# SoraKurihara/FFM

Measured on AMD Instinct MI355X. Metric: agent-steps/sec (whole node), 12×12 grid × 64k envs, 1/2/4/8 GPU, higher is better.
Workload: dtype f32; 1 GPU; ffm_core step, 12x12 room, 32 agents/env, 65536 envs/GPU, neumann, Philox seed 42, on-device auto-reset, steady state (envs desynchronised by a 1000-step untimed burn-in after reset); burn_in_steps=1000, map=12x12, agents_per_env=32, envs_per_gpu=65536, global_envs=65536, parallelism=env-sharded x1

## Files before the change

### ffm_amd/csrc/core_multi.hip

```cpp
#include <hip/hip_runtime.h>
#include <stdint.h>

#include "core_common.h"
#include "kernels.h"
#include "lane_common.h"
#include "episode_log.h"
#include "wave_reset.h"

namespace ffm {

namespace {

struct MultiCarve {
    size_t grid, tile, words, keys, posb, per_wave;
};

__host__ __device__ inline MultiCarve multi_carve(int PHW, int TS, int F) {
    MultiCarve c;
    size_t o = 0;
    c.grid = o;  o += a16((size_t)(2 * PHW) * 2);
    c.tile = o;  o += a16((size_t)(2 * TS) * 4);
    c.words = o; o += 64 * 8;
    c.keys = o;  o += a16((size_t)(F > 0 ? F : 1) * 8);
    c.posb = o;  o += 64 * 2;
// ... 115 lines not shown
                                   ((slot <= (uint32_t)NB ? slot : DirCodes::kNoDir) << 8));
            wave_sync();

            const int r = (int)slot_cell<NB>(slot, pp, PW);
            const bool req = slot <= (uint32_t)NB;
            const bool moving = req && r != pp;
            bool granted = req && !moving;
            {
                const int rt = moving ? r : pp;
                int m = 0, kr = 0, o = 0x7F;
#pragma unroll
                for (int s = 0; s < NB; s++) {
                    const uint32_t c = gk[rt - nb_dx<NB>(s) * PW - nb_dy<NB>(s)];
                    const bool is = (c & DirCodes::kAgent) != 0u && ((c >> 8) & 0xFu) == (uint32_t)s;
                    const int who = (int)(c & DirCodes::kIdx);
                    m += is ? 1 : 0;
                    kr += (is && who < al) ? 1 : 0;
                    o = (is && who < o) ? who : o;
                }
                if (moving) {
                    if (m == 1) {
                        granted = true;
                    } else {
                        const uint2 f = words[sub * 32 + o];
                        const int kk = philox_friction(f.x, f.y, (uint32_t)m, a.key0, a.key1, t, genv, (uint32_t)o);
                        granted = kk == kr;
                    }
                }
            }
            if (granted) __hip_atomic_fetch_add(dk + pp + dd0, 1.0f, __ATOMIC_RELAXED, __HIP_MEMORY_SCOPE_WAVEFRONT);
            const int np = granted ? r : pp;

            const bool keep = live && !(granted && to_exit);
            const unsigned long long km = __ballot(keep);
            const unsigned long long segm = sub ? 0xFFFFFFFF00000000ull : 0x00000000FFFFFFFFull;
            const int newidx = lanes_below(km & segm);
            const int newcnt = __popcll(km & segm);
            {
                const int n0 = __popcll(km & 0xFFFFFFFFull), n1 = __popcll(km >> 32);
                const int c0 = __builtin_amdgcn_readlane(cnt, 0), c1 = __builtin_amdgcn_readlane(cnt, 32);
                c_exits += (unsigned)((c0 - n0) + (nenv > 1 ? c1 - n1 : 0));
            }
            if (live) *mine = 0;
            if (keep) posb[sub * 32 + newidx] = (uint16_t)unpad(np, PW);
            const bool rs = a.auto_reset && env_ok && newcnt == 0;
            const unsigned long long rsm = __ballot(rs);
            if (rsm) {
                c_resets += (unsigned)(((rsm & 1ull) ? 1 : 0) + ((rsm >> 32) & 1ull ? 1 : 0));
                if (a.episodes && al == 0 && rs) a.episodes[e0 + sub] += 1;
                CoreStepArgs ak = a;
                ak.t = t;
                wave_sync();
                for (int s = 0; s < 2; s++)
                    if ((rsm >> (32 * s)) & 1ull) wave_reset_env(ak, ebase + (uint32_t)(e0 + s), keys, pfree, posb + s * 32, lane);
            }
            if (EPL && (rsm || !a.auto_reset))
                eplog_end_wave(a, env_ok && al == 0 && newcnt == 0 && cnt > 0, rs && al == 0, e0 + sub, t, lane);
            cnt = rs ? a.N : newcnt;
            wave_sync();
            cpos = posb[lane];

            auto stencil = [&](int tb, bool yl, bool yr, float4& out) {
                const float* p = tile + tb;
                float b[3][6];
#pragma unroll
                for (int dx = -1; dx <= 1; dx++) {
                    const float4 u = *reinterpret_cast<const float4*>(p + dx * W);
                    b[dx + 1][1] = a.c0 * u.x; b[dx + 1][2] = a.c0 * u.y;
                    b[dx + 1][3] = a.c0 * u.z; b[dx + 1][4] = a.c0 * u.w;
                    if (NB == 4 && dx != 0) continue;
                    b[dx + 1][0] = a.c0 * tile[yl ? 0 : tb + dx * W - 1];
                    b[dx + 1][5] = a.c0 * tile[yr ? 0 : tb + dx * W + 4];
                }
                float ov[4];
#pragma unroll
                for (int j = 0; j < 4; j++) {
                    float acc = b[1][j + 1];
#pragma unroll
                    for (int s = 0; s < NB; s++) {
                        const float tt = a.c1 * b[1 + nb_dx<NB>(s)][j + 1 + nb_dy<NB>(s)];
                        acc = acc + tt;
                    }
                    ov[j] = acc < 1e-4f ? 0.0f : acc;
                }
                out = make_float4(ov[0], ov[1], ov[2], ov[3]);
            };
            o0 = make_float4(0.f, 0.f, 0.f, 0.f);
            o1 = o0;
            if (tb0 >= 0) stencil(tb0, yl0, yr0, o0);
            if (tb1 >= 0) stencil(tb1, yl1, yr1, o1);
            {
                const bool r0 = (rsm & 1ull) != 0, r1 = (rsm >> 32) != 0;
                const bool z0 = zs0 == 0 ? r0 : (zs0 == 1 && r1), z1 = zs1 == 0 ? r0 : (zs1 == 1 && r1);
                if (z0) o0 = make_float4(0.f, 0.f, 0.f, 0.f);
                if (z1) o1 = make_float4(0.f, 0.f, 0.f, 0.f);
            }
            wave_sync();
            if (tb0 >= 0) *reinterpret_cast<float4*>(tile + tb0) = o0;
            if (tb1 >= 0) *reinterpret_cast<float4*>(tile + tb1) = o1;
            wave_sync();
        }

        __builtin_amdgcn_raw_buffer_store_b16((uint16_t)cpos, rp, (env_ok && al < cnt) ? (sub * A + al) * 2 : kOOB, 0, 0);
        __builtin_amdgcn_raw_buffer_store_b32((unsigned)cnt, rc, al == 0 ? sub * 4 : kOOB, 0, 0);
        buf_st4(rd, 16 * lane, o0);
        buf_st4(rd, 16 * lane + 1024, o1);
    }
// ... 50 lines not shown
```

### ffm_amd/csrc/engine.cpp

```cpp
#include "../../include/ffm_amd.h"

#include <hip/hip_runtime.h>

#include <algorithm>
#include <cmath>
#include <cstdio>
#include <cstdlib>
#include <cstring>
#include <string>
#include <vector>

#include "kernels.h"

namespace {
thread_local std::string g_err;
}

namespace ffm {
int set_error(int code, const std::string& msg) {
    g_err = msg;
    return code;
}
}

namespace {

int fail(int code, const std::string& msg) { return ffm::set_error(code, msg); }

#define HIP_TRY(expr)                                                                           \
    do {                                                                                        \
        hipError_t e_ = (expr);                                                                 \
        if (e_ != hipSuccess)                                                                   \
            return fail(FFM_E_HIP, std::string(#expr) + ": " + hipGetErrorString(e_));          \
    } while (0)

}

struct ffm_engine {
    ffm_engine_desc d{};
    int HW = 0, F = 0, K = 1, block = 256;
    bool f64 = false, mt = false;
    bool lane = false;
    bool wave = false;
    int wave_blocks = 0;
    int lane_blocks = 0;
    bool group = false;
    int group_blocks = 0;
    int group_g = 4;
    bool multi = false;
    int multi_blocks = 0;
    int fused = 1;
    float kS32 = 0, kD32 = 0, c0 = 0, c1 = 0;
    double kS64 = 0;
    uint32_t t = 0;
    uint8_t* d_map = nullptr;
    void* d_sff = nullptr;
    uint16_t* d_free = nullptr;
    uint16_t* d_free_padded = nullptr;
    unsigned char* d_stage = nullptr;
    size_t stage_bytes = 0;
    int stage_q4 = 0;
    uint16_t* d_pos = nullptr;
    int32_t* d_cnt = nullptr;
    float* d_dff = nullptr;
    float* d_tmp = nullptr;
    int32_t* d_eps = nullptr;
    unsigned long long* d_ctr = nullptr;
    size_t ctr_slots = 1;
    uint32_t* d_mt_np = nullptr;
    uint32_t* d_mt_py = nullptr;
    unsigned long long* d_dbg = nullptr;
    bool big = false;
    bool block_reset = false;
    unsigned char* d_scratch = nullptr;
    size_t scratch_stride = 0;
    ffm::CoreCapture cap{};
    uint32_t* d_ep_start = nullptr;
    int32_t* d_eplog = nullptr;
    unsigned long long* d_eplog_n = nullptr;
    long long eplog_cap = 0;
    unsigned long long* d_ephist = nullptr;
    int ephist_bins = 0;
    struct Shard {
        long long e0 = 0, n = 0;
        int blocks = 0, g = 4;
        size_t ctr0 = 0;
    };
    std::vector<Shard> shards;
    hipStream_t sh_stream[3] = {nullptr, nullptr, nullptr};
    hipEvent_t sh_fork = nullptr;
    hipEvent_t sh_end[3] = {nullptr, nullptr, nullptr};
};

static constexpr int kMaxStepShards = 4;
static constexpr int kDefaultStepShards = 2;

static size_t ep_sum_offset(int bins) { return ((size_t)bins + 15) & ~(size_t)15; }
static size_t ep_stats_words(int bins) { return ep_sum_offset(bins) + (size_t)ffm::kEpSumSlots * ffm::kEpSumStride; }

static void free_episode_log(ffm_engine* e, bool ep_start_too) {
    (void)hipFree(e->d_eplog);
    (void)hipFree(e->d_eplog_n);
    (void)hipFree(e->d_ephist);
    e->d_eplog = nullptr;
    e->d_eplog_n = nullptr;
    e->d_ephist = nullptr;
    e->eplog_cap = 0;
    e->ephist_bins = 0;
    if (ep_start_too) {
        (void)hipFree(e->d_ep_start);
        e->d_ep_start = nullptr;
    }
}

// ... 24 lines not shown
    (void)hipFree(e->d_free_padded);
    (void)hipFree(e->d_stage);
    (void)hipFree(e->d_pos);
    (void)hipFree(e->d_cnt);
    (void)hipFree(e->d_dff);
    (void)hipFree(e->d_tmp);
    (void)hipFree(e->d_eps);
    (void)hipFree(e->d_ctr);
    (void)hipFree(e->d_mt_np);
    (void)hipFree(e->d_mt_py);
    (void)hipFree(e->d_dbg);
    (void)hipFree(e->d_scratch);
    free_capture(e);
    free_episode_log(e, true);
    delete e;
}

int ffm_engine_create(const ffm_engine_desc* desc, ffm_engine** out) {
    if (!desc || !out) return fail(FFM_E_INVALID, "null argument");
    *out = nullptr;
    const ffm_engine_desc& d = *desc;
    if (d.abi_version != FFM_ABI_VERSION) return fail(FFM_E_INVALID, "abi_version mismatch");
    if (d.variant != FFM_VARIANT_CORE) return fail(FFM_E_UNSUPPORTED, "only FFM_VARIANT_CORE is built");
    if (d.H < 3 || d.W < 3 || (long long)d.H * d.W > 65536)
        return fail(FFM_E_INVALID, "map must be at least 3x3 and at most 65536 cells");
    if (!ffm::magic_div_ok((uint64_t)(d.H + 2) * (d.W + 2), (uint32_t)d.W + 2u))
        return fail(FFM_E_INVALID, "map too large for the kernels' magic divisors");
    if (!d.map || !d.sff) return fail(FFM_E_INVALID, "map and sff are required");
    if (d.neighborhood != 4 && d.neighborhood != 8) return fail(FFM_E_INVALID, "neighborhood must be 4 or 8");
    if (d.sff_dtype != FFM_SFF_F32 && d.sff_dtype != FFM_SFF_F64) return fail(FFM_E_INVALID, "sff_dtype");
    if (d.n_envs < 1) return fail(FFM_E_INVALID, "n_envs must be >= 1");
    if (d.agent_capacity < 1 || d.agent_capacity > 32767) return fail(FFM_E_INVALID, "agent_capacity");
    if (d.n_agents < 0 || d.n_agents > d.agent_capacity) return fail(FFM_E_INVALID, "n_agents > agent_capacity");
    if (d.rng_mode != FFM_RNG_PHILOX && d.rng_mode != FFM_RNG_MT) return fail(FFM_E_INVALID, "rng_mode");
    const int H = d.H, W = d.W, HW = H * W;
    std::vector<uint16_t> fl;
    for (int i = 0; i < HW; i++) {
        const int x = i / W, y = i % W;
        const bool border = x == 0 || y == 0 || x == H - 1 || y == W - 1;
        if (d.map[i] == 0) {
            if (border) return fail(FFM_E_INVALID, "free cell on the map border (walls must enclose the room)");
            fl.push_back((uint16_t)i);
        }
    }
    if (d.n_agents > (int)fl.size())
        return fail(FFM_E_INVALID, "Cannot take a larger sample than population when 'replace=False'");

    ffm_engine* e = new ffm_engine();
    e->d = d;
    e->d.map = nullptr;
    e->d.sff = nullptr;
    e->HW = HW;
    e->F = (int)fl.size();
    e->f64 = d.sff_dtype == FFM_SFF_F64;
    e->mt = d.rng_mode == FFM_RNG_MT;
    e->kS32 = (float)(-d.k_S);
    e->kD32 = (float)d.k_D;
    e->kS64 = -d.k_S;
    e->c0 = (float)((1.0 - d.decay) * (1.0 - d.diffuse));
    e->c1 = (float)(d.decay * (1.0 - d.diffuse) / (double)d.neighborhood);

    auto cleanup = [&](int rc) {
        release(e);
        return rc;
    };
    hipError_t he = hipSetDevice(d.device);
    if (he != hipSuccess) return cleanup(fail(FFM_E_HIP, std::string("hipSetDevice: ") + hipGetErrorString(he)));

    const int A = d.agent_capacity;
    const bool reset_lds = !e->mt && d.auto_reset;
    const int EW = A <= 32 ? 2 : 1;
    const bool lane_ok = !e->mt && !e->f64 && A <= 32 && W % 4 == 0 && HW <= 256 &&
                         ((long long)d.n_envs + 7) * HW * 4 < (1ll << 31);
    e->group = (d.envs_per_block == 0 || d.envs_per_block == -3) && lane_ok && ffm::core_group_supported(H, W) &&
               ffm::core_group_smem_bytes(H, W, e->F, 4) <= 64 * 1024;
    e->multi = lane_ok && ffm::core_multi_smem_bytes(H, W, e->F, 4) <= 64 * 1024;
    e->lane = !e->group && (d.envs_per_block == 0 || d.envs_per_block == -2) && lane_ok &&
              ffm::core_lane_smem_bytes(H, W, e->F, 4) <= 64 * 1024;
    e->wave = !e->lane && !e->group && (d.envs_per_block == 0 || d.envs_per_block == -1) && A <= 64 && !e->f64 && W % 4 == 0 && EW * HW <= 512 &&
              ffm::core_wave_smem_bytes(H, W, A, e->F, e->mt, reset_lds, 4) <= 64 * 1024;
    e->block = A > 256 ? 512 : 256;
    if (const char* bs = getenv("FFM_BLOCK_BS"))
        if (atoi(bs) == 256 || atoi(bs) == 512) e->block = atoi(bs);
    int K = d.envs_per_block > 0 ? d.envs_per_block : std::max(1, 256 / A);
    if (e->mt) K = 1;
    while (K > 1 && ffm::core_block_smem_bytes(H, W, A, K, e->F, e->f64, e->mt, reset_lds) > 64 * 1024) K--;
    e->K = K;
    e->big = !e->wave && !e->lane && !e->group &&
             ((size_t)(H + 2) * (W + 2) > 65535 ||
              ffm::core_block_smem_bytes(H, W, A, K, e->F, e->f64, e->mt, reset_lds) > 64 * 1024);
    if (e->big) e->K = 1;
    auto al16 = [](size_t x) { return (x + 15) & ~(size_t)15; };
    const size_t wave_reset_lds = al16(8 * (size_t)std::max(1, e->F)) + al16(2 * (size_t)std::max(1, d.n_agents)) +
                                  al16(2 * (size_t)std::max(1, e->F));
    e->block_reset = !e->mt && wave_reset_lds > 64 * 1024;

    const size_t E = (size_t)d.n_envs;
    const int PW = W + 2, PHW = (H + 2) * PW;
    const size_t sff_bytes = (size_t)PHW * (e->f64 ? 8 : 4);
    std::vector<uint8_t> pmap((size_t)PHW, 2);
    std::vector<double> psff64((size_t)PHW, 0.0);
    std::vector<float> psff32((size_t)PHW, 0.0f);
    for (int x = 0; x < H; x++)
        for (int y = 0; y < W; y++) {
            const int i = x * W + y, p = (x + 1) * PW + y + 1;
            pmap[p] = d.map[i] == 0 ? 0 : d.map[i] == 3 ? 3 : 2;
// ... 146 lines not shown
    }
    if (he == hipSuccess) he = hipMemset(e->d_pos, 0xFF, pos_bytes);
    if (he == hipSuccess) he = hipMemset(e->d_cnt, 0, Ep * 4);
    if (he == hipSuccess) he = hipMemset(e->d_dff, 0, Ep * HW * 4);
    if (he == hipSuccess) he = hipMemset(e->d_eps, 0, E * 4);
    if (he == hipSuccess) he = hipMemset(e->d_ctr, 0, e->ctr_slots * 32);
    if (he == hipSuccess) he = hipMemset(e->d_dbg, 0, 128);
    if (he == hipSuccess && e->mt) he = hipMemset(e->d_mt_np, 0, E * 625 * 4);
    if (he == hipSuccess && e->mt) he = hipMemset(e->d_mt_py, 0, E * 625 * 4);
    if (he != hipSuccess) return cleanup(fail(FFM_E_HIP, std::string("init: ") + hipGetErrorString(he)));
    *out = e;
    return FFM_OK;
}

int ffm_engine_destroy(ffm_engine* e) {
    if (!e) return FFM_OK;
    (void)hipSetDevice(e->d.device);
    (void)hipDeviceSynchronize();
    release(e);
    return FFM_OK;
}

static ffm::CoreStepArgs make_args(ffm_engine* e) {
    ffm::CoreStepArgs a{};
    a.mW = ffm::magic_div((uint32_t)e->d.W);
    a.mPW = ffm::magic_div((uint32_t)e->d.W + 2u);
    a.H = e->d.H;
    a.W = e->d.W;
    a.HW = e->HW;
    a.A = e->d.agent_capacity;
    a.K = e->K;
    a.E = e->d.n_envs;
    a.env_base = e->d.env_base;
    a.pos = e->d_pos;
    a.cnt = e->d_cnt;
    a.dff = e->d_dff;
    a.episodes = e->d_eps;
    a.counters = e->d_ctr;
    a.pmap = e->d_map;
    a.psff = e->d_sff;
    a.kS32 = e->kS32;
    a.kD32 = e->kD32;
    a.kS64 = e->kS64;
    a.c0 = e->c0;
    a.c1 = e->c1;
    a.key0 = (uint32_t)e->d.seed;
    a.key1 = (uint32_t)(e->d.seed >> 32);
    a.t = e->t;
    a.auto_reset = e->d.auto_reset && !e->mt;
    a.N = e->d.n_agents;
    a.free_list = e->d_free;
    a.free_padded = e->d_free_padded;
    a.F = e->F;
    a.stage = e->d_stage;
    a.stage_q4 = e->stage_q4;
    a.mt_np = e->d_mt_np;
    a.mt_py = e->d_mt_py;
    a.dbg = e->d_dbg;
    a.scratch = e->big ? e->d_scratch : nullptr;
    a.scratch_stride = e->scratch_stride;
    a.ep_start = e->d_ep_start;
    a.eplog = e->d_eplog;
    a.eplog_n = e->d_eplog_n;
    a.eplog_cap = e->eplog_cap;
    a.ephist = e->d_ephist;
    a.ephist_bins = e->ephist_bins;
    a.epsum = e->d_ephist ? e->d_ephist + ep_sum_offset(e->ephist_bins) : nullptr;
    return a;
}

static int shards_in_effect(const ffm_engine* e) {
    if (e->shards.size() <= 1 || e->cap.n_sel != 0 || (e->fused > 1 && e->multi)) return 1;
    return (int)e->shards.size();
}

static int step_sharded(ffm_engine* e, int32_t n_steps, hipStream_t s) {
    const size_t S = e->shards.size();
    const int A = e->d.agent_capacity;
    HIP_TRY(hipEventRecord(e->sh_fork, s));
    for (size_t k = 1; k < S; k++) HIP_TRY(hipStreamWaitEvent(e->sh_stream[k - 1], e->sh_fork, 0));
    const ffm::CoreStepArgs base = make_args(e);
    hipError_t he = hipSuccess;
    int done = 0;
    for (; done < n_steps && he == hipSuccess; done++) {
        for (size_t k = 0; k < S && he == hipSuccess; k++) {
            const ffm_engine::Shard& sh = e->shards[k];
            ffm::CoreStepArgs a = base;
            a.t = e->t + (uint32_t)done;
            a.E = sh.n;
            a.env_base = base.env_base + sh.e0;
            a.pos = base.pos + sh.e0 * A;
            a.cnt = base.cnt + sh.e0;
            a.dff = base.dff + sh.e0 * e->HW;
            a.episodes = base.episodes + sh.e0;
            if (base.ep_start) a.ep_start = base.ep_start + sh.e0;
            a.counters = base.counters + 4 * sh.ctr0;
            a.no_step_count = k != 0;
            he = ffm::launch_core_group(a, e->d.neighborhood, sh.blocks, k ? e->sh_stream[k - 1] : s, sh.g);
        }
    }
    hipError_t hj = hipSuccess;
    for (size_t k = 1; k < S; k++) {
        hipError_t h1 = hipEventRecord(e->sh_end[k - 1], e->sh_stream[k - 1]);
        if (h1 == hipSuccess) h1 = hipStreamWaitEvent(s, e->sh_end[k - 1], 0);
        if (h1 != hipSuccess) hj = h1;
    }
// ... 336 lines not shown

int ffm_engine_get_counters(ffm_engine* e, uint64_t* counters, void* stream) {
    if (!e || !counters) return fail(FFM_E_INVALID, "null argument");
    hipStream_t s = (hipStream_t)stream;
    std::vector<unsigned long long> c(e->ctr_slots * 4);
    HIP_TRY(hipMemcpyAsync(c.data(), e->d_ctr, e->ctr_slots * 32, hipMemcpyDeviceToHost, s));
    HIP_TRY(hipStreamSynchronize(s));
    for (int i = 0; i < 4; i++) counters[i] = 0;
    for (size_t j = 0; j < e->ctr_slots; j++)
        for (int i = 0; i < 4; i++) counters[i] += c[j * 4 + i];
    return FFM_OK;
}

int ffm_engine_device_buffers(ffm_engine* e, ffm_device_buffers* out) {
    if (!e || !out) return fail(FFM_E_INVALID, "null argument");
    out->positions = e->d_pos;
    out->counts = e->d_cnt;
    out->dff = e->d_dff;
    out->episodes = e->d_eps;
    out->counters = reinterpret_cast<uint64_t*>(e->d_ctr);
    out->mt_np = e->d_mt_np;
    out->mt_py = e->d_mt_py;
    out->counter_slots = (int64_t)e->ctr_slots;
    return FFM_OK;
}

int ffm_engine_get_step_index(ffm_engine* e, uint32_t* t) {
    if (!e || !t) return fail(FFM_E_INVALID, "null argument");
    *t = e->t;
    return FFM_OK;
}

int ffm_engine_set_step_index(ffm_engine* e, uint32_t t) {
    if (!e) return fail(FFM_E_INVALID, "null engine");
    e->t = t;
    return FFM_OK;
}

int ffm_debug_read(ffm_engine* e, uint64_t* out, int n) {
    if (!e || !out || n < 0 || n > 16) return fail(FFM_E_INVALID, "bad args");
    HIP_TRY(hipMemcpy(out, e->d_dbg, (size_t)n * 8, hipMemcpyDeviceToHost));
    return FFM_OK;
}

int ffm_debug_stage_image(ffm_engine* e, void* out, int64_t cap, int64_t* n) {
    if (!e || !n || cap < 0) return fail(FFM_E_INVALID, "bad args");
    *n = (int64_t)e->stage_bytes;
    if (!out || e->stage_bytes == 0) return FFM_OK;
    if (cap < (int64_t)e->stage_bytes) return fail(FFM_E_INVALID, "stage_image: buffer too small (*n holds the size)");
    HIP_TRY(hipMemcpy(out, e->d_stage, e->stage_bytes, hipMemcpyDeviceToHost));
    return FFM_OK;
}

int ffm_debug_launch_info(ffm_engine* e, int32_t* out, int n) {
    if (!e || !out || n < 0 || n > 9) return fail(FFM_E_INVALID, "bad args");
    const int kernel = e->group ? 0 : e->lane ? 1 : e->wave ? 2 : e->big ? 4 : 3;
    const long long E = e->d.n_envs;
    const int S = shards_in_effect(e);
    const int32_t step_blocks = e->group ? e->group_blocks : e->lane ? e->lane_blocks : e->wave ? e->wave_blocks
                                                                                              : (int32_t)((E + e->K - 1) / e->K);
    const int32_t v[9] = {
        kernel,
        e->group ? e->group_g : 0,
        step_blocks,
        e->K,
        kernel <= 2 ? 256 : e->big ? 1024 : e->block,
        e->multi ? 1 : 0,
        e->multi ? e->multi_blocks : 0,
        S,
        S > 1 ? e->shards[0].blocks : step_blocks,
    };
    for (int i = 0; i < n; i++) out[i] = v[i];
    return FFM_OK;
}

int ffm_np_expf_device(const float* x, float* y, int64_t n, void* stream) {
    HIP_TRY(ffm::launch_np_expf(x, y, n, (hipStream_t)stream));
    return FFM_OK;
}

}
```

### ffm_amd/csrc/kernels.h

```cpp
#pragma once
#include <hip/hip_runtime.h>
#include <stddef.h>
#include <stdint.h>

namespace ffm {

__host__ __device__ inline uint32_t magic_div(uint32_t d) { return (uint32_t)((0x100000000ull + d - 1) / d); }
__host__ __device__ inline bool magic_div_ok(uint64_t n_end, uint32_t d) { return n_end * (uint64_t)d <= 0x100000000ull; }

struct CoreStepArgs {
    int H, W, HW;
    uint32_t mW, mPW;
    int A;
    int K;
    long long E;
    long long env_base;
    uint16_t* pos;
    int* cnt;
    float* dff;
    int* episodes;
    unsigned long long* counters;
    const uint8_t* pmap;
    const void* psff;
    float kS32, kD32;
    double kS64;
    float c0, c1;
    uint32_t key0, key1;
    uint32_t t;
    int auto_reset, N;
    const uint16_t* free_list;
    const uint16_t* free_padded;
    int F;
    uint32_t* mt_np;
    uint32_t* mt_py;
    unsigned long long* dbg;
    unsigned char* scratch;
    size_t scratch_stride;
    int no_step_count;
    const void* stage;
    int stage_q4;
    uint32_t* ep_start;
    int* eplog;
    unsigned long long* eplog_n;
    long long eplog_cap;
    unsigned long long* ephist;
    int ephist_bins;
    unsigned long long* epsum;
};

constexpr int kEpSumSlots = 64, kEpSumStride = 16;

struct CoreCapture {
    const int* envs;
    const int* phase;
    int* state;
    int* meta;
    uint16_t* cells;
    unsigned long long* n;
    long long cap;
    int n_sel, period;
};

size_t core_wave_smem_bytes(int H, int W, int A, int F, bool mt, bool reset, int waves);
size_t core_block_smem_bytes(int H, int W, int A, int K, int F, bool f64, bool mt, bool reset);
hipError_t launch_core_wave(const CoreStepArgs& a, int nb, bool mt, int blocks, hipStream_t s);
int core_wave_blocks_per_cu(const CoreStepArgs& a, int nb, bool mt);
size_t core_lane_smem_bytes(int H, int W, int F, int waves);
hipError_t launch_core_lane(const CoreStepArgs& a, int nb, int blocks, hipStream_t s);
int core_lane_blocks_per_cu(const CoreStepArgs& a, int nb);
int core_lane_max_pairs_per_wave();
size_t core_group_smem_bytes(int H, int W, int F, int waves, int G = 4);
bool core_group_supported(int H, int W);
int core_group_max_iters();
size_t core_group_stage_bytes(int H, int W, int F);
int core_group_stage_q4(int H, int W, int F);
void core_group_stage_build(int H, int W, int F, const uint8_t* pmap, const float* psff, float kS32,
                            const uint16_t* free_padded, unsigned char* out);
int core_group_pick_envs(const CoreStepArgs& a, int nb, long long E, int cus);
hipError_t launch_core_group(const CoreStepArgs& a, int nb, int blocks, hipStream_t s, int G);
int core_group_blocks_per_cu(const CoreStepArgs& a, int nb, int G);
size_t core_multi_smem_bytes(int H, int W, int F, int waves);
hipError_t launch_core_multi(const CoreStepArgs& a, int nb, int nsteps, int blocks, hipStream_t s);
int core_multi_blocks_per_cu(const CoreStepArgs& a, int nb);
hipError_t launch_core_block(const CoreStepArgs& a, int nb, bool f64, bool mt, int block, hipStream_t s);
hipError_t launch_core_reset(const CoreStepArgs& a, hipStream_t s, const uint8_t* mask = nullptr);
size_t core_big_scratch_bytes(int H, int W, int A, int F, bool mt);
hipError_t launch_core_block_reset(const CoreStepArgs& a, hipStream_t s, const uint8_t* mask = nullptr);
hipError_t launch_update_dff(const float* src, float* dst, long long E, int H, int W, int nb, float c0,
                             float c1, hipStream_t s);
hipError_t launch_core_capture_init(const CoreStepArgs& a, const CoreCapture& c, hipStream_t s);
hipError_t launch_core_capture(const CoreStepArgs& a, const CoreCapture& c, hipStream_t s);
// ... 4 lines not shown
```

### ffm_amd/csrc/wave_reset.h

```cpp
#pragma once
#include "core_common.h"
#include "kernels.h"

namespace ffm {

__device__ __forceinline__ unsigned long long readlane64(unsigned long long v, int l) {
    const uint32_t lo = (uint32_t)__builtin_amdgcn_readlane((int)(uint32_t)v, l);
    const uint32_t hi = (uint32_t)__builtin_amdgcn_readlane((int)(uint32_t)(v >> 32), l);
    return ((unsigned long long)hi << 32) | lo;
}

template <int PWK = 0, bool SMALL = false>
__device__ inline void wave_reset_env(const CoreStepArgs& a, uint32_t genv, unsigned long long* keys, const uint16_t* fl,
                               uint16_t* gpos, int lane) {
    const int PW = PWK > 0 ? PWK : a.W + 2;
    const int F = a.F, N = a.N;
    if (SMALL || F <= 128) {
        const int j0 = lane, j1 = lane + 64;
        const unsigned long long k0 =
            j0 < F ? ((unsigned long long)reset_key(a.key0, a.key1, a.t, genv, (uint32_t)j0) << 32) | (unsigned)j0
                   : ~0ull;
        const unsigned long long k1 =
            j1 < F ? ((unsigned long long)reset_key(a.key0, a.key1, a.t, genv, (uint32_t)j1) << 32) | (unsigned)j1
                   : ~0ull;
        if (j0 < F) keys[j0] = k0;
        if (j1 < F) keys[j1] = k1;
        if (lane == 0 && (F & 1)) keys[F] = ~0ull;
        wave_sync();
        int r0 = 0, r1 = 0;
        const ulonglong2* kv = reinterpret_cast<const ulonglong2*>(keys);
#pragma unroll 8
        for (int q = 0; q < (F + 1) / 2; q++) {
            const ulonglong2 p = kv[q];
            r0 += (p.x < k0 ? 1 : 0) + (p.y < k0 ? 1 : 0);
            r1 += (p.x < k1 ? 1 : 0) + (p.y < k1 ? 1 : 0);
        }
        if (j0 < F && r0 < N) gpos[r0] = (uint16_t)unpad(fl[j0], PW);
        if (j1 < F && r1 < N) gpos[r1] = (uint16_t)unpad(fl[j1], PW);
        wave_sync();
        return;
    }
    uint32_t T = reset_threshold(N, F);
    int C = 0;
    for (int attempt = 0; attempt < 2; attempt++) {
        C = 0;
        for (int j0 = 0; j0 < F; j0 += 64) {
            const int j = j0 + lane;
            uint32_t k = 0;
            bool cand = false;
            if (j < F) {
                k = reset_key(a.key0, a.key1, a.t, genv, (uint32_t)j);
                cand = k <= T;
            }
            const unsigned long long m = __ballot(cand);
            if (cand) keys[C + lanes_below(m)] = ((unsigned long long)k << 32) | (unsigned)j;
            C += __popcll(m);
        }
        if (C >= N || T == 0xFFFFFFFFu) break;
        T = 0xFFFFFFFFu;
    }
    wave_sync();
    for (int i = lane; i < C; i += 64) {
        const unsigned long long ki = keys[i];
        int rank = 0;
        for (int q = 0; q < C; q++) rank += keys[q] < ki ? 1 : 0;
        if (rank < N) gpos[rank] = (uint16_t)unpad(fl[(int)(ki & 0xFFFFu)], PW);
    }
    wave_sync();
}

}
```

### ffm_amd/engine.py

```python
from __future__ import annotations

import ctypes as C
import os
import random as _pyrandom

import numpy as np

_HERE = os.path.dirname(os.path.abspath(__file__))
LIB_PATH = os.environ.get("FFM_LIB_PATH") or os.path.join(_HERE, "_lib", "libffm_amd.so")

ABI_VERSION = 2
OK, E_INVALID, E_HIP, E_NOMEM, E_UNSUPPORTED = 0, -1, -2, -3, -4
VARIANT_CORE = 0
RNG_PHILOX, RNG_MT = 0, 1
SFF_F32, SFF_F64 = 0, 1

EXPORTED = [
    "ffm_last_error", "ffm_abi_version", "ffm_engine_create", "ffm_engine_destroy",
    "ffm_engine_reset", "ffm_engine_reset_envs", "ffm_engine_step", "ffm_engine_update_dff", "ffm_engine_set_state",
    "ffm_engine_get_state", "ffm_engine_set_mt_state", "ffm_engine_get_mt_state",
    "ffm_engine_get_counters", "ffm_engine_device_buffers", "ffm_engine_get_step_index",
    "ffm_engine_set_step_index", "ffm_engine_set_fused_steps", "ffm_np_expf_device",
    "ffm_engine_set_trajectory_capture", "ffm_engine_drain_trajectory",
    "ffm_engine_set_episode_log", "ffm_engine_drain_episodes", "ffm_engine_get_episode_stats",
    "ffm_debug_stage_image",
    "ffm_learner_create", "ffm_learner_destroy", "ffm_learner_reset", "ffm_learner_reset_envs", "ffm_learner_step",
    "ffm_learner_set_state", "ffm_learner_get_state", "ffm_learner_get_episodes",
    "ffm_learner_set_mt_state", "ffm_learner_get_mt_state", "ffm_learner_get_counters",
    "ffm_learner_set_epsilon", "ffm_learner_set_v_default", "ffm_learner_table_size",
    "ffm_learner_export_table", "ffm_learner_import_table", "ffm_learner_get_step_index",
    "ffm_learner_set_step_index", "ffm_learner_step_local", "ffm_learner_step_apply", "ffm_learner_step_end",
    "ffm_learner_delta_export", "ffm_learner_delta_merge", "ffm_learner_set_placement",
    "ffm_learner_set_epsilon_schedule", "ffm_learner_set_epsilon_phase", "ffm_learner_drain_episodes",
    "ffm_learner_set_trajectory_capture", "ffm_learner_drain_trajectory",
    "ffm_learner_delta_export_async", "ffm_learner_delta_merge_async", "ffm_learner_set_sync_period",
    "ffm_learner_apply_due", "ffm_learner_dense_buffers", "ffm_learner_dense_adopt",
    "ffm_learner_tiled_buffers", "ffm_learner_step_tiled_local", "ffm_learner_step_tiled_apply",
    "ffm_learner_set_external_sync", "ffm_learner_flush_begin", "ffm_learner_flush_end",
    "ffm_learner_set_tile_owners", "ffm_learner_owner_buffers", "ffm_learner_step_owner_local",
    "ffm_learner_step_owner_v", "ffm_learner_step_owner_h", "ffm_learner_step_owner_end",
    "ffm_learner_set_epsilon_stride", "ffm_learner_set_episode_caps", "ffm_learner_set_owner_capacity",
    "ffm_learner_set_owner_send_buffer", "ffm_learner_set_owner_output_buffers", "ffm_learner_set_h_extra",
]

VARIANT_AC, VARIANT_UNIFIED, VARIANT_ACTOR_ONLY, VARIANT_TRAINED = 1, 2, 3, 4
LEARN_MODES = {"critic_only": 0, "actor_only": 1, "both": 2}
TABLE_V, TABLE_H = 0, 1


class EngineDesc(C.Structure):
    _fields_ = [
        ("abi_version", C.c_int32), ("variant", C.c_int32),
        ("H", C.c_int32), ("W", C.c_int32),
        ("map", C.c_void_p), ("sff", C.c_void_p), ("sff_dtype", C.c_int32),
        ("neighborhood", C.c_int32),
        ("k_S", C.c_double), ("k_D", C.c_double), ("diffuse", C.c_double), ("decay", C.c_double),
        ("n_envs", C.c_int64), ("agent_capacity", C.c_int32), ("n_agents", C.c_int32),
        ("rng_mode", C.c_int32), ("auto_reset", C.c_int32), ("seed", C.c_uint64),
        ("env_base", C.c_int64), ("device", C.c_int32), ("envs_per_block", C.c_int32),
    ]


class LearnDesc(C.Structure):
    _fields_ = [
        ("mode", C.c_int32), ("k_A", C.c_double),
        ("alpha_v", C.c_double), ("alpha_h", C.c_double), ("gamma", C.c_double),
        ("exit_reward", C.c_double), ("step_penalty", C.c_double), ("collision_penalty", C.c_double),
        ("epsilon", C.c_double), ("v_default", C.c_double),
        ("block_size", C.c_int32), ("max_steps", C.c_int32),
        ("log2_v_capacity", C.c_int32), ("log2_h_capacity", C.c_int32),
        ("eps_start", C.c_double), ("eps_end", C.c_double), ("eps_offset", C.c_double), ("eps_span", C.c_double),
    ]


class OwnerBuffers(C.Structure):
    _fields_ = [
        ("world", C.c_int32), ("rank", C.c_int32),
        ("send_recs", C.c_void_p), ("send_rec_capacity", C.c_int64),
        ("send_hdr", C.c_void_p), ("hdr_stride", C.c_int64),
        ("counts", C.c_void_p),
        ("v_slot", C.c_void_p), ("v_val", C.c_void_p), ("h_key", C.c_void_p), ("h_q", C.c_void_p),
        ("out_counts", C.c_void_p), ("v_capacity", C.c_int64), ("h_capacity", C.c_int64),
        ("tsum", C.c_void_p), ("tsum_count", C.c_int64),
    ]


class DeviceBuffers(C.Structure):
    _fields_ = [
        ("positions", C.c_void_p), ("counts", C.c_void_p), ("dff", C.c_void_p),
        ("episodes", C.c_void_p), ("counters", C.c_void_p),
        ("mt_np", C.c_void_p), ("mt_py", C.c_void_p), ("counter_slots", C.c_int64),
    ]


_lib = None


def load_library():
    global _lib
    if _lib is not None:
        return _lib
    if not os.path.exists(LIB_PATH):
        raise ImportError(
            f"ffm_amd HIP library not found at {LIB_PATH}; build it with "
            "`python -m ffm_amd.build` (hipcc --offload-arch=gfx950)")
    L = C.CDLL(LIB_PATH)
    P, i32, i64 = C.c_void_p, C.c_int32, C.c_int64
    L.ffm_last_error.restype = C.c_char_p
    L.ffm_abi_version.restype = C.c_int
    L.ffm_engine_create.argtypes = [C.POINTER(EngineDesc), C.POINTER(P)]
    L.ffm_engine_destroy.argtypes = [P]
    L.ffm_engine_reset.argtypes = [P, P]
    L.ffm_engine_reset_envs.argtypes = [P, P, P]
    L.ffm_engine_step.argtypes = [P, i32, P]
    L.ffm_engine_update_dff.argtypes = [P, P]
    L.ffm_engine_set_state.argtypes = [P, i64, i64, P, P, P, P]
    L.ffm_engine_get_state.argtypes = [P, i64, i64, P, P, P, P]
    L.ffm_engine_set_mt_state.argtypes = [P, i64, P, i32, P, i32, P]
    L.ffm_engine_get_mt_state.argtypes = [P, i64, P, C.POINTER(i32), P, C.POINTER(i32), P]
    L.ffm_engine_get_counters.argtypes = [P, P, P]
    L.ffm_engine_device_buffers.argtypes = [P, C.POINTER(DeviceBuffers)]
    L.ffm_engine_get_step_index.argtypes = [P, C.POINTER(C.c_uint32)]
    L.ffm_engine_set_step_index.argtypes = [P, C.c_uint32]
    L.ffm_engine_set_fused_steps.argtypes = [P, i32]
    L.ffm_engine_set_trajectory_capture.argtypes = [P, P, P, i32, i32, i64, P]
    L.ffm_engine_drain_trajectory.argtypes = [P, P, P, i64, C.POINTER(i64), C.POINTER(i64), P]
    L.ffm_engine_set_episode_log.argtypes = [P, i64, i32, P]
    L.ffm_engine_drain_episodes.argtypes = [P, P, i64, C.POINTER(i64), C.POINTER(i64), P]
    L.ffm_engine_get_episode_stats.argtypes = [P, P, i32, P, i32, P]
    L.ffm_np_expf_device.argtypes = [P, P, i64, P]
    L.ffm_debug_stage_image.argtypes = [P, P, i64, C.POINTER(i64)]
    L.ffm_debug_launch_info.argtypes = [P, P, C.c_int]
    L.ffm_debug_launch_info.restype = C.c_int
    L.ffm_learner_create.argtypes = [C.POINTER(EngineDesc), C.POINTER(LearnDesc), C.POINTER(P)]
    L.ffm_learner_destroy.argtypes = [P]
    L.ffm_learner_reset.argtypes = [P, P]
    L.ffm_learner_reset_envs.argtypes = [P, P, P]
    L.ffm_learner_step.argtypes = [P, i32, P]
    L.ffm_learner_set_state.argtypes = [P, i64, i64, P, P, P, P]
    L.ffm_learner_get_state.argtypes = [P, i64, i64, P, P, P, P]
    L.ffm_learner_get_episodes.argtypes = [P, i64, i64, P, P, P]
    L.ffm_learner_set_mt_state.argtypes = [P, i64, P, i32, P, i32, P]
    L.ffm_learner_get_mt_state.argtypes = [P, i64, P, C.POINTER(i32), P, C.POINTER(i32), P]
    L.ffm_learner_get_counters.argtypes = [P, P, P]
    L.ffm_learner_set_epsilon.argtypes = [P, C.c_double]
    L.ffm_learner_set_v_default.argtypes = [P, C.c_double, P]
    L.ffm_learner_set_h_extra.argtypes = [P, C.c_int64, C.c_double, C.c_double, C.c_int32]
    L.ffm_learner_table_size.argtypes = [P, i32, C.POINTER(i64), P]
    L.ffm_learner_export_table.argtypes = [P, i32, P, P, i64, C.POINTER(i64), P]
    L.ffm_learner_import_table.argtypes = [P, i32, P, P, i64, P]
    L.ffm_learner_get_step_index.argtypes = [P, C.POINTER(C.c_uint32)]
    L.ffm_learner_set_step_index.argtypes = [P, C.c_uint32]
    L.ffm_learner_step_local.argtypes = [P, P]
    L.ffm_learner_step_apply.argtypes = [P, i32, P]
    L.ffm_learner_step_end.argtypes = [P, P]
    L.ffm_learner_delta_export.argtypes = [P, i32, P, P, i64, C.POINTER(i64), P]
    L.ffm_learner_delta_merge.argtypes = [P, i32, P, P, i64, P]
    L.ffm_learner_set_placement.argtypes = [P, P, i32, i32]
    L.ffm_learner_set_epsilon_schedule.argtypes = [P, C.c_double, C.c_double, C.c_double, C.c_double]
    L.ffm_learner_set_epsilon_phase.argtypes = [P, i32]
    L.ffm_learner_set_epsilon_stride.argtypes = [P, i64]
    L.ffm_learner_set_episode_caps.argtypes = [P, P, i64]
    L.ffm_learner_drain_episodes.argtypes = [P, P, i64, C.POINTER(i64), C.POINTER(i64), P]
    L.ffm_learner_set_trajectory_capture.argtypes = [P, P, P, i32, i32, i64, P]
    L.ffm_learner_delta_export_async.argtypes = [P, i32, P, P, i64, P, P]
    L.ffm_learner_delta_merge_async.argtypes = [P, i32, P, P, P, i64, P]
    L.ffm_learner_set_sync_period.argtypes = [P, i32]
    L.ffm_learner_apply_due.argtypes = [P, C.POINTER(i32)]
    L.ffm_learner_dense_buffers.argtypes = [P, i32, C.POINTER(P), C.POINTER(i64), C.POINTER(P), C.POINTER(i64)]
    L.ffm_learner_dense_adopt.argtypes = [P, i32, P, P]
    L.ffm_learner_tiled_buffers.argtypes = [P, C.POINTER(P), C.POINTER(i64), C.POINTER(P), C.POINTER(i64)]
    L.ffm_learner_step_tiled_local.argtypes = [P, P]
    L.ffm_learner_step_tiled_apply.argtypes = [P, P, P, i64, P]
    L.ffm_learner_drain_trajectory.argtypes = [P, P, P, i64, C.POINTER(i64), C.POINTER(i64), P]
    L.ffm_learner_set_tile_owners.argtypes = [P, i32, i32]
    L.ffm_learner_owner_buffers.argtypes = [P, C.POINTER(OwnerBuffers)]
    L.ffm_learner_step_owner_local.argtypes = [P, P]
    L.ffm_learner_set_owner_capacity.argtypes = [P, i64, i64, i64]
    L.ffm_learner_step_owner_v.argtypes = [P, P, P, i64, P]
    L.ffm_learner_set_owner_send_buffer.argtypes = [P, P]
    L.ffm_learner_set_owner_output_buffers.argtypes = [P, P, P, P, P, P, P]
    L.ffm_learner_step_owner_h.argtypes = [P, P, P, P, i64, P]
    L.ffm_learner_step_owner_end.argtypes = [P, P, P, P, i64, P, i64, P]
    L.ffm_learner_set_external_sync.argtypes = [P, i32]
# ... 284 lines not shown
            raise ValueError("MT19937 keys must have 624 words")
        _check(self._L.ffm_engine_set_mt_state(self._h, env, _ptr(nk), int(np_pos), _ptr(pk),
                                               int(py_pos), _stream_handle(stream)))

    def get_mt_state(self, env: int, stream=None):
        nk = np.empty(624, np.uint32)
        pk = np.empty(624, np.uint32)
        npos, ppos = C.c_int32(), C.c_int32()
        _check(self._L.ffm_engine_get_mt_state(self._h, env, _ptr(nk), C.byref(npos), _ptr(pk),
                                               C.byref(ppos), _stream_handle(stream)))
        return nk, int(npos.value), pk, int(ppos.value)

    def load_rng_from(self, env: int, np_rs: np.random.RandomState | None = None,
                      py_r: _pyrandom.Random | None = None):
        st = (np_rs if np_rs is not None else np.random.mtrand._rand).get_state(legacy=True)
        ps = (py_r if py_r is not None else _pyrandom._inst).getstate()
        self.set_mt_state(env, st[1], st[2], np.asarray(ps[1][:624], np.uint32), ps[1][624])

    def store_rng_to(self, env: int, np_rs: np.random.RandomState | None = None,
                     py_r: _pyrandom.Random | None = None):
        nk, npos, pk, ppos = self.get_mt_state(env)
        rs = np_rs if np_rs is not None else np.random.mtrand._rand
        st = rs.get_state(legacy=True)
        rs.set_state(("MT19937", nk, npos, st[3], st[4]))
        r = py_r if py_r is not None else _pyrandom._inst
        ps = r.getstate()
        r.setstate((ps[0], tuple(int(w) for w in pk) + (ppos,), ps[2]))

    def counters(self, stream=None) -> dict:
        c = np.zeros(4, np.uint64)
        _check(self._L.ffm_engine_get_counters(self._h, _ptr(c), _stream_handle(stream)))
        return {"agent_steps": int(c[0]), "exits": int(c[1]), "resets": int(c[2]), "steps": int(c[3])}

    def device_buffers(self) -> dict:
        b = DeviceBuffers()
        _check(self._L.ffm_engine_device_buffers(self._h, C.byref(b)))
        return {k: b.__getattribute__(k) for k, _ in DeviceBuffers._fields_}

    def launch_info(self) -> dict:
        v = np.zeros(9, np.int32)
        _check(self._L.ffm_debug_launch_info(self._h, _ptr(v), len(v)))
        return {"kernel": ("group", "lane", "wave", "block", "block_scratch")[int(v[0])], "group_g": int(v[1]),
                "blocks": int(v[2]), "K": int(v[3]), "block_size": int(v[4]), "multi": bool(v[5]),
                "multi_blocks": int(v[6]), "step_shards": int(v[7]), "shard_blocks": int(v[8])}

    def stage_image(self) -> np.ndarray:
        n = C.c_int64()
        _check(self._L.ffm_debug_stage_image(self._h, None, 0, C.byref(n)))
        out = np.zeros(n.value, np.uint8)
        if n.value:
            _check(self._L.ffm_debug_stage_image(self._h, _ptr(out), n.value, C.byref(n)))
        return out

    @property
    def step_index(self) -> int:
        t = C.c_uint32()
        _check(self._L.ffm_engine_get_step_index(self._h, C.byref(t)))
        return int(t.value)

    @step_index.setter
    def step_index(self, t: int):
        _check(self._L.ffm_engine_set_step_index(self._h, int(t) & 0xFFFFFFFF))


def np_expf_device(x_dev_ptr: int, y_dev_ptr: int, n: int, stream=None):
    L = load_library()
    _check(L.ffm_np_expf_device(x_dev_ptr, y_dev_ptr, n, _stream_handle(stream)))


LEARN_DEFAULTS = {
    "ac": {"k_S": 10, "k_D": 1, "diffuse": 0.2, "decay": 0.2, "neighborhood": "neumann", "alpha_v": 0.1,
           "gamma": 0.95, "exit_reward": 100.0, "step_penalty": 0.0, "collision_penalty": -1.0,
           "block_size": 3},
    "unified": {"k_S": 10, "k_D": 1, "k_A": 10, "diffuse": 0.2, "decay": 0.2, "neighborhood": "neumann",
                "alpha_v": 0.1, "gamma": 0.95, "exit_reward": 100.0, "step_penalty": 0.0,
                "collision_penalty": -1.0, "block_size": 5, "alpha_h": 0.1, "epsilon": 0.0},
    "actor_only": {"k_D": 1, "k_A": 10, "diffuse": 0.2, "decay": 0.2, "neighborhood": "neumann",
                   "alpha_v": 0.1, "gamma": 0.95, "exit_reward": 100.0, "step_penalty": 0.0,
                   "collision_penalty": -1.0, "alpha_h": 0.1, "epsilon": 0.0},
    "trained": {"k_D": 1, "k_A": 10, "diffuse": 0.2, "decay": 0.2, "neighborhood": "neumann", "block_size": 5},
}
_LEARN_VARIANTS = {"ac": VARIANT_AC, "unified": VARIANT_UNIFIED, "actor_only": VARIANT_ACTOR_ONLY,
                   "trained": VARIANT_TRAINED}


class Learner:

    def __init__(self, map_array, sff, variant: str, n_envs: int, n_agents: int,
                 agent_capacity: int | None = None, mode: str | None = None, params: dict | None = None,
                 rng: str = "philox", seed: int = 42, auto_reset: bool = True, max_steps: int = 0,
                 env_base: int = 0, device: int = 0, log2_v_capacity: int = 0, log2_h_capacity: int = 0):
        L = load_library()
        if variant not in _LEARN_VARIANTS:
            raise ValueError(f"variant must be one of {sorted(_LEARN_VARIANTS)}")
        p = {**LEARN_DEFAULTS[variant], **(params or {})}
        self.params, self.variant = p, variant
        self.mode = mode or ("actor_only" if variant == "actor_only" else "critic_only")
        if variant == "unified" and self.mode not in LEARN_MODES:
            raise ValueError(f"learning_mode must be one of {list(LEARN_MODES)}")
        self.map = np.ascontiguousarray(map_array, dtype=np.uint8)
        if self.map.ndim != 2:
            raise ValueError("map must be 2-D")
        self.H, self.W = self.map.shape
        sff = np.asarray(sff)
        if sff.shape != self.map.shape:
            raise ValueError("sff shape must equal map shape")
# ... 429 lines not shown
```

### include/ffm_amd.h

```cpp
#ifndef FFM_AMD_H
#define FFM_AMD_H

#include <stdint.h>

#ifdef __cplusplus
extern "C" {
#endif

#define FFM_ABI_VERSION 2

enum {
    FFM_OK = 0,
    FFM_E_INVALID = -1,
    FFM_E_HIP = -2,
    FFM_E_NOMEM = -3,
    FFM_E_UNSUPPORTED = -4
};

enum {
    FFM_VARIANT_CORE = 0,
    FFM_VARIANT_AC = 1,
    FFM_VARIANT_UNIFIED = 2,
    FFM_VARIANT_ACTOR_ONLY = 3,
    FFM_VARIANT_TRAINED = 4
// ... 146 lines not shown
    int64_t send_rec_capacity;
    uint32_t* send_hdr;
    int64_t hdr_stride;
    int64_t* counts;
    uint32_t* v_slot;
    double* v_val;
    uint32_t* h_key;
    int64_t* h_q;
    int64_t* out_counts;
    int64_t v_capacity, h_capacity;
    double* tsum;
    int64_t tsum_count;
} ffm_owner_buffers;
int ffm_learner_set_tile_owners(ffm_learner* l, int32_t world, int32_t rank);
int ffm_learner_set_owner_capacity(ffm_learner* l, int64_t rec_capacity, int64_t v_capacity, int64_t h_capacity);
int ffm_learner_owner_buffers(ffm_learner* l, ffm_owner_buffers* b);
int ffm_learner_step_owner_local(ffm_learner* l, void* stream);
int ffm_learner_set_owner_send_buffer(ffm_learner* l, void* d_buf);
int ffm_learner_set_owner_output_buffers(ffm_learner* l, uint32_t* v_slot, double* v_val, int64_t* v_count,
                                         uint32_t* h_key, int64_t* h_q, int64_t* h_count);
int ffm_learner_step_owner_v(ffm_learner* l, const void* d_recs, const uint32_t* d_hdrs, int64_t src_stride,
                             void* stream);
int ffm_learner_step_owner_h(ffm_learner* l, const uint32_t* d_v_slot, const double* d_v_val,
                             const int64_t* d_v_counts, int64_t v_stride, void* stream);
int ffm_learner_step_owner_end(ffm_learner* l, const uint32_t* d_h_key, const int64_t* d_h_q,
                               const int64_t* d_h_counts, int64_t h_stride, const double* d_tsum_all,
                               int64_t tsum_stride, void* stream);
int ffm_learner_set_sync_period(ffm_learner* l, int32_t period);
int ffm_learner_apply_due(ffm_learner* l, int32_t* due);
int ffm_learner_set_external_sync(ffm_learner* l, int32_t on);
int ffm_learner_flush_begin(ffm_learner* l, int32_t* pending);
int ffm_learner_flush_end(ffm_learner* l, void* stream);
int ffm_learner_dense_buffers(ffm_learner* l, int32_t which, int64_t** d_acc, int64_t* acc_count,
                              uint32_t** d_present, int64_t* present_words);
int ffm_learner_dense_adopt(ffm_learner* l, int32_t which, const uint32_t* d_union, void* stream);
int ffm_learner_set_placement(ffm_learner* l, const uint16_t* cells, int32_t count, int32_t n_agents);
int ffm_learner_set_epsilon_schedule(ffm_learner* l, double eps_start, double eps_end, double eps_offset,
                                     double eps_span);
int ffm_learner_set_epsilon_phase(ffm_learner* l, int32_t period);
int ffm_learner_set_epsilon_stride(ffm_learner* l, int64_t stride);
int ffm_learner_set_episode_caps(ffm_learner* l, const int32_t* caps, int64_t n);
int ffm_learner_drain_episodes(ffm_learner* l, int32_t* records, int64_t cap, int64_t* n, int64_t* dropped,
                               void* stream);
int ffm_learner_set_trajectory_capture(ffm_learner* l, const int32_t* envs, const int32_t* phases, int32_t n_sel,
                                       int32_t period, int64_t capacity_rows, void* stream);
int ffm_learner_drain_trajectory(ffm_learner* l, int32_t* meta, uint16_t* cells, int64_t cap, int64_t* n,
                                 int64_t* dropped, void* stream);
int ffm_learner_get_step_index(ffm_learner* l, uint32_t* t);
int ffm_learner_set_step_index(ffm_learner* l, uint32_t t);

int ffm_np_expf_device(const float* x, float* y, int64_t n, void* stream);

int ffm_debug_stage_image(ffm_engine* eng, void* out, int64_t cap, int64_t* n);

#ifdef __cplusplus
}
#endif
#endif
```

Before: 51.91 billion agent-steps/s.

## Rank only threshold-filtered candidate keys in wave reset sampling

Episode reset samples N free cells by ranking random keys over every free cell. The change first keeps only keys below a threshold sized so that about M candidates (N plus a margin) pass. When at least N and at most 64 survive, only those are compacted and ranked, which shrinks the O(F) comparison loop. Otherwise it falls back to the full ranking, so the sampled set should match the original. The multi-env kernel path explicitly keeps the old behaviour via template args, so only other wave reset callers use the new path.

New measurement: 54.46 billion agent-steps/s (median of 6 runs). 1.05x the previous value.

```diff
diff --git a/ffm_amd/csrc/core_multi.hip b/ffm_amd/csrc/core_multi.hip
--- a/ffm_amd/csrc/core_multi.hip
+++ b/ffm_amd/csrc/core_multi.hip
@@ -191,7 +191,8 @@
                 ak.t = t;
                 wave_sync();
                 for (int s = 0; s < 2; s++)
-                    if ((rsm >> (32 * s)) & 1ull) wave_reset_env(ak, ebase + (uint32_t)(e0 + s), keys, pfree, posb + s * 32, lane);
+                    if ((rsm >> (32 * s)) & 1ull)
+                        wave_reset_env<0, false, false>(ak, ebase + (uint32_t)(e0 + s), keys, pfree, posb + s * 32, lane);
             }
             if (EPL && (rsm || !a.auto_reset))
                 eplog_end_wave(a, env_ok && al == 0 && newcnt == 0 && cnt > 0, rs && al == 0, e0 + sub, t, lane);
diff --git a/ffm_amd/csrc/engine.cpp b/ffm_amd/csrc/engine.cpp
--- a/ffm_amd/csrc/engine.cpp
+++ b/ffm_amd/csrc/engine.cpp
@@ -60,6 +60,8 @@
     unsigned char* d_stage = nullptr;
     size_t stage_bytes = 0;
     int stage_q4 = 0;
+    int reset_m = 0;
+    uint32_t reset_thr = 0;
     uint16_t* d_pos = nullptr;
     int32_t* d_cnt = nullptr;
     float* d_dff = nullptr;
@@ -190,6 +192,13 @@
     e->d.sff = nullptr;
     e->HW = HW;
     e->F = (int)fl.size();
+    {
+        const int N = d.n_agents, F = e->F;
+        int M = std::min(F, N + std::max(8, (N + 1) / 2));
+        if (const char* ov = std::getenv("FFM_RESET_CANDIDATES")) M = std::max(0, std::min(F, std::atoi(ov)));
+        e->reset_m = M;
+        e->reset_thr = M == 0 ? 0u : M == F ? 0xFFFFFFFFu : (uint32_t)(((uint64_t)M << 32) / (uint64_t)F);
+    }
     e->f64 = d.sff_dtype == FFM_SFF_F64;
     e->mt = d.rng_mode == FFM_RNG_MT;
     e->kS32 = (float)(-d.k_S);
@@ -442,6 +451,7 @@
     a.free_list = e->d_free;
     a.free_padded = e->d_free_padded;
     a.F = e->F;
+    a.reset_thr = e->reset_thr;
     a.stage = e->d_stage;
     a.stage_q4 = e->stage_q4;
     a.mt_np = e->d_mt_np;
@@ -884,6 +894,13 @@
     return FFM_OK;
 }
 
+int ffm_debug_reset_candidates(ffm_engine* e, int32_t* m, uint32_t* thr) {
+    if (!e || !m || !thr) return fail(FFM_E_INVALID, "bad args");
+    *m = e->reset_m;
+    *thr = e->reset_thr;
+    return FFM_OK;
+}
+
 int ffm_debug_launch_info(ffm_engine* e, int32_t* out, int n) {
     if (!e || !out || n < 0 || n > 9) return fail(FFM_E_INVALID, "bad args");
     const int kernel = e->group ? 0 : e->lane ? 1 : e->wave ? 2 : e->big ? 4 : 3;
diff --git a/ffm_amd/csrc/kernels.h b/ffm_amd/csrc/kernels.h
--- a/ffm_amd/csrc/kernels.h
+++ b/ffm_amd/csrc/kernels.h
@@ -37,6 +37,7 @@
     unsigned char* scratch;
     size_t scratch_stride;
     int no_step_count;
+    uint32_t reset_thr;
     const void* stage;
     int stage_q4;
     uint32_t* ep_start;
diff --git a/ffm_amd/csrc/wave_reset.h b/ffm_amd/csrc/wave_reset.h
--- a/ffm_amd/csrc/wave_reset.h
+++ b/ffm_amd/csrc/wave_reset.h
@@ -10,7 +10,7 @@
     return ((unsigned long long)hi << 32) | lo;
 }
 
-template <int PWK = 0, bool SMALL = false>
+template <int PWK = 0, bool SMALL = false, bool CAND = true>
 __device__ inline void wave_reset_env(const CoreStepArgs& a, uint32_t genv, unsigned long long* keys, const uint16_t* fl,
                                uint16_t* gpos, int lane) {
     const int PW = PWK > 0 ? PWK : a.W + 2;
@@ -23,6 +23,28 @@
         const unsigned long long k1 =
             j1 < F ? ((unsigned long long)reset_key(a.key0, a.key1, a.t, genv, (uint32_t)j1) << 32) | (unsigned)j1
                    : ~0ull;
+        if (CAND) {
+            const bool c0 = (uint32_t)(k0 >> 32) < a.reset_thr, c1 = (uint32_t)(k1 >> 32) < a.reset_thr;
+            const unsigned long long m0 = __ballot(c0), m1 = __ballot(c1);
+            const int C0 = __popcll(m0), C = C0 + __popcll(m1);
+            if (C >= N && C <= 64) {
+                if (c0) keys[lanes_below(m0)] = k0;
+                if (c1) keys[C0 + lanes_below(m1)] = k1;
+                if (lane == 0 && (C & 1)) keys[C] = ~0ull;
+                wave_sync();
+                const unsigned long long ki = lane < C ? keys[lane] : ~0ull;
+                int r = 0;
+                const ulonglong2* kv = reinterpret_cast<const ulonglong2*>(keys);
+#pragma unroll 4
+                for (int q = 0; q < (C + 1) / 2; q++) {
+                    const ulonglong2 p = kv[q];
+                    r += (p.x < ki ? 1 : 0) + (p.y < ki ? 1 : 0);
+                }
+                if (lane < C && r < N) gpos[r] = (uint16_t)unpad(fl[(int)(ki & 0xFFu)], PW);
+                wave_sync();
+                return;
+            }
+        }
         if (j0 < F) keys[j0] = k0;
         if (j1 < F) keys[j1] = k1;
         if (lane == 0 && (F & 1)) keys[F] = ~0ull;
diff --git a/ffm_amd/engine.py b/ffm_amd/engine.py
--- a/ffm_amd/engine.py
+++ b/ffm_amd/engine.py
@@ -23,7 +23,7 @@
     "ffm_engine_set_step_index", "ffm_engine_set_fused_steps", "ffm_np_expf_device",
     "ffm_engine_set_trajectory_capture", "ffm_engine_drain_trajectory",
     "ffm_engine_set_episode_log", "ffm_engine_drain_episodes", "ffm_engine_get_episode_stats",
-    "ffm_debug_stage_image",
+    "ffm_debug_stage_image", "ffm_debug_reset_candidates",
     "ffm_learner_create", "ffm_learner_destroy", "ffm_learner_reset", "ffm_learner_reset_envs", "ffm_learner_step",
     "ffm_learner_set_state", "ffm_learner_get_state", "ffm_learner_get_episodes",
     "ffm_learner_set_mt_state", "ffm_learner_get_mt_state", "ffm_learner_get_counters",
@@ -130,6 +130,7 @@
     L.ffm_engine_get_episode_stats.argtypes = [P, P, i32, P, i32, P]
     L.ffm_np_expf_device.argtypes = [P, P, i64, P]
     L.ffm_debug_stage_image.argtypes = [P, P, i64, C.POINTER(i64)]
+    L.ffm_debug_reset_candidates.argtypes = [P, C.POINTER(i32), C.POINTER(C.c_uint32)]
     L.ffm_debug_launch_info.argtypes = [P, P, C.c_int]
     L.ffm_debug_launch_info.restype = C.c_int
     L.ffm_learner_create.argtypes = [C.POINTER(EngineDesc), C.POINTER(LearnDesc), C.POINTER(P)]
@@ -520,6 +521,11 @@
             _check(self._L.ffm_debug_stage_image(self._h, _ptr(out), n.value, C.byref(n)))
         return out
 
+    def reset_candidates(self) -> dict:
+        m, thr = C.c_int32(), C.c_uint32()
+        _check(self._L.ffm_debug_reset_candidates(self._h, C.byref(m), C.byref(thr)))
+        return {"M": int(m.value), "thr": int(thr.value)}
+
     @property
     def step_index(self) -> int:
         t = C.c_uint32()
diff --git a/include/ffm_amd.h b/include/ffm_amd.h
--- a/include/ffm_amd.h
+++ b/include/ffm_amd.h
@@ -222,6 +222,7 @@
 int ffm_np_expf_device(const float* x, float* y, int64_t n, void* stream);
 
 int ffm_debug_stage_image(ffm_engine* eng, void* out, int64_t cap, int64_t* n);
+int ffm_debug_reset_candidates(ffm_engine* eng, int32_t* m, uint32_t* thr);
 
 #ifdef __cplusplus
 }
```
